# lhaippp/DMHomo

Measured on AMD Instinct MI355X. Metric: sampled images/sec (128x128, s_step=32), higher is better.
Workload: dtype f32; 1 GPU; DGM CFG-Unet dim=64 128x128 bs=25/GPU s_step=32 cond_scale=3 (BASELINE configs[1]); global_batch=25, cfg_mode=streams, hip_graph=True, weights=seeded random init

## Files before the change

### dmhomo_amd/csrc/attention.hip

```cpp
#include "common.h"

typedef float floatx16 __attribute__((ext_vector_type(16)));

#define LA_NS 128
#define LA_PART (32 + 32 + 1024)

__global__ __launch_bounds__(256) void linattn_context_kernel(const float* __restrict__ qkv,
                                                              float* __restrict__ partial, int n, int nsplit,
                                                              const int32_t* __restrict__ rows) {
  const int jb = blockIdx.x / nsplit, sp = blockIdx.x % nsplit;
  if (rows && jb >= rows[0]) return;
  const int b = dmh_rows_phys(rows, jb);
  const int lane = threadIdx.x & 63, h = threadIdx.x >> 6;
  const int d = lane & 31, half = lane >> 5;
  const int p0 = sp * LA_NS;
  const float* base = qkv + (size_t)b * n * 384;

  float kr[LA_NS / 2], vr[LA_NS / 2];
  const float* kp = base + (size_t)p0 * 384 + 128 + h * 32 + d + (size_t)half * 384;
#pragma unroll
  for (int i = 0; i < LA_NS / 2; ++i) {
    const int pix = p0 + 2 * i + half;
    const bool ok = pix < n;
    const float* q = ok ? kp + (size_t)i * 768 : kp;
    const float kv = q[0], vv = q[128];
    kr[i] = ok ? kv : -INFINITY;
    vr[i] = ok ? vv : 0.f;
  }
  float m = -INFINITY;
#pragma unroll
  for (int i = 0; i < LA_NS / 2; ++i) m = fmaxf(m, kr[i]);
  m = fmaxf(m, __shfl_xor(m, 32));
  float s = 0.f;
#pragma unroll
  for (int i = 0; i < LA_NS / 2; ++i) {
    kr[i] = __expf(kr[i] - m);
    s += kr[i];
  }
  s += __shfl_xor(s, 32);

  floatx16 acc;
#pragma unroll
  for (int r = 0; r < 16; ++r) acc[r] = 0.f;
#pragma unroll
  for (int i = 0; i < LA_NS / 2; ++i) acc = __builtin_amdgcn_mfma_f32_32x32x2f32(kr[i], vr[i], acc, 0, 0, 0);
  float* out = partial + ((size_t)(b * nsplit + sp) * 4 + h) * LA_PART;
  if (half == 0) {
    out[d] = m;
    out[32 + d] = s;
  }
#pragma unroll
  for (int r = 0; r < 16; ++r) {
    const int row = (r & 3) + 8 * (r >> 2) + 4 * half;
    out[64 + row * 32 + d] = acc[r];
  }
}

__global__ __launch_bounds__(1024) void linattn_merge_kernel(const float* __restrict__ partial,
                                                             float* __restrict__ ctx, int n, int nsplit,
                                                             float* __restrict__ ms, const int32_t* __restrict__ rows) {
  if (rows && (int)(blockIdx.x >> 2) >= rows[0]) return;
  const int b = dmh_rows_phys(rows, blockIdx.x >> 2), h = blockIdx.x & 3;
  const int bh = b * 4 + h;
  const int d = threadIdx.x >> 5, e = threadIdx.x & 31;
  const float* base = partial + ((size_t)b * nsplit * 4 + h) * LA_PART;
  const size_t stride = (size_t)4 * LA_PART;
  float M = -INFINITY;
#pragma unroll 8
  for (int sp = 0; sp < nsplit; ++sp) M = fmaxf(M, base[sp * stride + d]);
  float S = 0.f, acc = 0.f;
#pragma unroll 8
  for (int sp = 0; sp < nsplit; ++sp) {
    const float w = expf(base[sp * stride + d] - M);
    S = fmaf(base[sp * stride + 32 + d], w, S);
    acc = fmaf(base[sp * stride + 64 + d * 32 + e], w, acc);
  }
  ctx[(size_t)bh * 1024 + d * 32 + e] = acc / S / (float)n;
  if (ms && e == 0) {
    ms[((size_t)bh * 32 + d) * 2 + 0] = M;
    ms[((size_t)bh * 32 + d) * 2 + 1] = S;
  }
}

#define LA_TILES 4
__global__ __launch_bounds__(256) void linattn_apply_kernel(const float* __restrict__ qkv,
                                                            const float* __restrict__ ctx, float* __restrict__ out,
                                                            int n, int nblk, float scale,
                                                            const int32_t* __restrict__ rows) {
  const int jb = blockIdx.x / nblk, blk = blockIdx.x % nblk;
  if (rows && jb >= rows[0]) return;
  const int b = dmh_rows_phys(rows, jb);
  const int lane = threadIdx.x & 63, h = threadIdx.x >> 6;
  const int i = lane & 31, half = lane >> 5;
  const float* cb = ctx + ((size_t)(b * 4 + h)) * 1024;
  float bf[16];
#pragma unroll
  for (int s = 0; s < 16; ++s) bf[s] = cb[(half * 16 + s) * 32 + i];
  const float* base = qkv + (size_t)b * n * 384;
  float* ob = out + (size_t)b * n * 128;
  for (int tI = 0; tI < LA_TILES; ++tI) {
    const int p0 = (blk * LA_TILES + tI) * 32;
    if (p0 >= n) break;
    const int pix = p0 + i;
    float q[16];
    if (pix < n) {
      const float* qp = base + (size_t)pix * 384 + h * 32 + half * 16;
#pragma unroll
      for (int s4 = 0; s4 < 4; ++s4) {
        const float4 t = ld4(qp + s4 * 4);
        q[s4 * 4 + 0] = t.x;
        q[s4 * 4 + 1] = t.y;
        q[s4 * 4 + 2] = t.z;
        q[s4 * 4 + 3] = t.w;
      }
    } else {
#pragma unroll
      for (int s = 0; s < 16; ++s) q[s] = 0.f;
    }
    float m = q[0];
#pragma unroll
    for (int s = 1; s < 16; ++s) m = fmaxf(m, q[s]);
    m = fmaxf(m, __shfl_xor(m, 32));
    float sum = 0.f;
#pragma unroll
    for (int s = 0; s < 16; ++s) {
      q[s] = expf(q[s] - m);
      sum += q[s];
    }
    sum += __shfl_xor(sum, 32);
    floatx16 acc;
#pragma unroll
    for (int r = 0; r < 16; ++r) acc[r] = 0.f;
#pragma unroll
    for (int s = 0; s < 16; ++s) {
      const float a = (q[s] / sum) * scale;
      acc = __builtin_amdgcn_mfma_f32_32x32x2f32(a, bf[s], acc, 0, 0, 0);
    }
#pragma unroll
    for (int r = 0; r < 16; ++r) {
      const int row = (r & 3) + 8 * (r >> 2) + 4 * half;
      if (p0 + row < n) ob[(size_t)(p0 + row) * 128 + h * 32 + i] = acc[r];
    }
  }
}

__global__ __launch_bounds__(256) void attention_kernel(const float* __restrict__ qkv, float* __restrict__ out, int n,
                                                        int qtiles, float scale, const int32_t* __restrict__ rows) {
  const int wid = blockIdx.x * 4 + (threadIdx.x >> 6);
  const int lane = threadIdx.x & 63;
  const int i = lane & 31, half = lane >> 5;
  const int qt = wid % qtiles;
  const int bh = wid / qtiles;
  const int h = bh & 3;
  if (rows && (bh >> 2) >= rows[0]) return;
  const int b = dmh_rows_phys(rows, bh >> 2);
  const float* base = qkv + (size_t)b * n * 384;
  const int q0 = qt * 32;

  float qf[16];
  {
    const int qi = q0 + i;
    if (qi < n) {
      const float* qp = base + (size_t)qi * 384 + h * 32 + half * 16;
#pragma unroll
      for (int s4 = 0; s4 < 4; ++s4) {
        const float4 t = ld4(qp + s4 * 4);
        qf[s4 * 4 + 0] = t.x * scale;
        qf[s4 * 4 + 1] = t.y * scale;
        qf[s4 * 4 + 2] = t.z * scale;
        qf[s4 * 4 + 3] = t.w * scale;
      }
    } else {
#pragma unroll
      for (int s = 0; s < 16; ++s) qf[s] = 0.f;
    }
  }
  floatx16 oacc;
#pragma unroll
  for (int r = 0; r < 16; ++r) oacc[r] = 0.f;
  float mrun = -INFINITY, lrun = 0.f;

  for (int k0 = 0; k0 < n; k0 += 32) {
    float kf[16];
    const int ki = k0 + i;
    if (ki < n) {
      const float* kp = base + (size_t)ki * 384 + 128 + h * 32 + half * 16;
#pragma unroll
      for (int s4 = 0; s4 < 4; ++s4) {
        const float4 t = ld4(kp + s4 * 4);
        kf[s4 * 4 + 0] = t.x;
        kf[s4 * 4 + 1] = t.y;
        kf[s4 * 4 + 2] = t.z;
        kf[s4 * 4 + 3] = t.w;
      }
    } else {
#pragma unroll
      for (int s = 0; s < 16; ++s) kf[s] = 0.f;
    }
    floatx16 sacc;
#pragma unroll
    for (int r = 0; r < 16; ++r) sacc[r] = 0.f;
#pragma unroll
    for (int s = 0; s < 16; ++s) sacc = __builtin_amdgcn_mfma_f32_32x32x2f32(kf[s], qf[s], sacc, 0, 0, 0);
    float tmax = -INFINITY;
#pragma unroll
    for (int r = 0; r < 16; ++r) {
      const int key = k0 + (r & 3) + 8 * (r >> 2) + 4 * half;
      if (key >= n) sacc[r] = -INFINITY;
      tmax = fmaxf(tmax, sacc[r]);
    }
    tmax = fmaxf(tmax, __shfl_xor(tmax, 32));
    const float mnew = fmaxf(mrun, tmax);
    const float alpha = expf(mrun - mnew);
    float psum = 0.f;
#pragma unroll
    for (int r = 0; r < 16; ++r) {
      sacc[r] = expf(sacc[r] - mnew);
      psum += sacc[r];
    }
    psum += __shfl_xor(psum, 32);
    lrun = fmaf(lrun, alpha, psum);
    mrun = mnew;
#pragma unroll
    for (int r = 0; r < 16; ++r) oacc[r] *= alpha;
#pragma unroll
    for (int r = 0; r < 16; ++r) {
      const int key = k0 + (r & 3) + 8 * (r >> 2) + 4 * half;
      const float vv = (key < n) ? base[(size_t)key * 384 + 256 + h * 32 + i] : 0.f;
      oacc = __builtin_amdgcn_mfma_f32_32x32x2f32(vv, sacc[r], oacc, 0, 0, 0);
    }
  }
  const int qi = q0 + i;
  if (qi < n) {
    float* op = out + ((size_t)b * n + qi) * 128 + h * 32;
    const float inv = 1.0f / lrun;
#pragma unroll
    for (int g4 = 0; g4 < 4; ++g4) {
      float4 o;
      o.x = oacc[g4 * 4 + 0] * inv;
      o.y = oacc[g4 * 4 + 1] * inv;
      o.z = oacc[g4 * 4 + 2] * inv;
      o.w = oacc[g4 * 4 + 3] * inv;
      st4(op + 8 * g4 + 4 * half, o);
    }
  }
}

extern "C" int dmh_linattn_splits(int n) { return dmh_dims_ok({n}, 1, 1 << 26) ? cdiv(n, LA_NS) : -1; }

extern "C" int64_t dmh_linattn_partial_floats(int B, int n) {
  if (!dmh_dims_ok({B}) || !dmh_dims_ok({n}, 1, 1 << 26)) return -1;
  return (int64_t)B * dmh_linattn_splits(n) * 4 * LA_PART;
}

extern "C" int dmh_linattn_context(const float* qkv, float* partial, int B, int n, const int32_t* rows, void* stream) {
  DMH_REQUIRE(qkv && partial && B > 0 && n > 0, "dmh_linattn_context: bad arguments");
  const int ns = dmh_linattn_splits(n);
  hipLaunchKernelGGL(linattn_context_kernel, dim3(B * ns), dim3(256), 0, (hipStream_t)stream, qkv, partial, n, ns, rows);
  DMH_CHECK_LAUNCH("dmh_linattn_context");
  return DMH_OK;
}

extern "C" int dmh_linattn_merge(const float* partial, float* ctx, int B, int n, const int32_t* rows, void* stream) {
  DMH_REQUIRE(partial && ctx && B > 0 && n > 0, "dmh_linattn_merge: bad arguments");
  hipLaunchKernelGGL(linattn_merge_kernel, dim3(B * 4), dim3(1024), 0, (hipStream_t)stream, partial, ctx, n,
                     dmh_linattn_splits(n), (float*)nullptr, rows);
  DMH_CHECK_LAUNCH("dmh_linattn_merge");
  return DMH_OK;
}

extern "C" int dmh_linattn_merge_n(const float* partial, float* ctx, int B, int n, int nsplit, const int32_t* rows,
                                   void* stream) {
  DMH_REQUIRE(partial && ctx && B > 0 && n > 0 && nsplit > 0, "dmh_linattn_merge_n: bad arguments");
  hipLaunchKernelGGL(linattn_merge_kernel, dim3(B * 4), dim3(1024), 0, (hipStream_t)stream, partial, ctx, n, nsplit,
                     (float*)nullptr, rows);
  DMH_CHECK_LAUNCH("dmh_linattn_merge_n");
  return DMH_OK;
}

extern "C" int dmh_linattn_merge_ms(const float* partial, float* ctx, float* ms, int B, int n, void* stream) {
  DMH_REQUIRE(partial && ctx && ms && B > 0 && n > 0, "dmh_linattn_merge_ms: bad arguments");
  hipLaunchKernelGGL(linattn_merge_kernel, dim3(B * 4), dim3(1024), 0, (hipStream_t)stream, partial, ctx, n,
                     dmh_linattn_splits(n), ms, (const int32_t*)nullptr);
  DMH_CHECK_LAUNCH("dmh_linattn_merge_ms");
  return DMH_OK;
}

extern "C" int dmh_linattn_apply(const float* qkv, const float* ctx, float* out, int B, int n, float scale,
                                 const int32_t* rows, void* stream) {
  DMH_REQUIRE(qkv && ctx && out && B > 0 && n > 0, "dmh_linattn_apply: bad arguments");
  const int nblk = cdiv(n, 32 * LA_TILES);
  hipLaunchKernelGGL(linattn_apply_kernel, dim3(B * nblk), dim3(256), 0, (hipStream_t)stream, qkv, ctx, out, n, nblk,
                     scale, rows);
  DMH_CHECK_LAUNCH("dmh_linattn_apply");
  return DMH_OK;
}

extern "C" int dmh_attention(const float* qkv, float* out, int B, int n, float scale, const int32_t* rows, void* stream) {
  DMH_REQUIRE(qkv && out && B > 0 && n > 0, "dmh_attention: bad arguments");
  const int qtiles = cdiv(n, 32);
  const int waves = B * 4 * qtiles;
  hipLaunchKernelGGL(attention_kernel, dim3(waves / 4), dim3(256), 0, (hipStream_t)stream, qkv, out, n, qtiles, scale, rows);
  DMH_CHECK_LAUNCH("dmh_attention");
  return DMH_OK;
}
```

Baseline: 89.75 images/s.

## Stage K/V tiles in LDS shared by four query waves in attention

The attention kernel now groups four 32-query waves of the same batch-head into one workgroup. K and V for 256 keys are loaded cooperatively with vectorized float4 global loads into padded LDS, and every wave reuses them, so each wave no longer re-reads K and strided scalar V from global memory. The LDS stores are split into stages with barriers so compute on early stages can begin while later stages are still being written. The exchange is extra LDS use, since the launch raises the dynamic shared memory limit, plus block-wide barriers and a higher register count from holding the prefetched K/V.

```diff
diff --git a/dmhomo_amd/csrc/attention.hip b/dmhomo_amd/csrc/attention.hip
--- a/dmhomo_amd/csrc/attention.hip
+++ b/dmhomo_amd/csrc/attention.hip
@@ -1,3 +1,4 @@
+#include <algorithm>
 #include "common.h"
 
 typedef float floatx16 __attribute__((ext_vector_type(16)));
@@ -144,90 +145,137 @@
   }
 }
 
+#define AT_KB 256
+#define AT_KP 36
+#define AT_ROW (AT_KP + 32)
+#define AT_STAGES 4
+#define AT_SK (AT_KB / AT_STAGES)
+
+__device__ __forceinline__ float at_half_max(float v) {
+  unsigned o;
+  const unsigned a = dmh_xor32(__float_as_uint(v), &o);
+  return fmaxf(__uint_as_float(a), __uint_as_float(o));
+}
+__device__ __forceinline__ float at_half_sum(float v) {
+  unsigned o;
+  const unsigned a = dmh_xor32(__float_as_uint(v), &o);
+  return __uint_as_float(a) + __uint_as_float(o);
+}
+
+__device__ __forceinline__ void at_tile(const float* Ks, const float* Vs, int kt, int k0, int n, int i, int half,
+                                        const float (&qf)[16], floatx16& oacc, float& mrun, float& lrun) {
+  float kf[16];
+  const float* kp = Ks + (kt + i) * AT_KP + half * 16;
+#pragma unroll
+  for (int s4 = 0; s4 < 4; ++s4) {
+    const float4 t = ld4(kp + s4 * 4);
+    kf[s4 * 4 + 0] = t.x;
+    kf[s4 * 4 + 1] = t.y;
+    kf[s4 * 4 + 2] = t.z;
+    kf[s4 * 4 + 3] = t.w;
+  }
+  float vf[16];
+#pragma unroll
+  for (int r = 0; r < 16; ++r) vf[r] = Vs[(kt + (r & 3) + 8 * (r >> 2) + 4 * half) * 32 + i];
+  floatx16 sacc;
+#pragma unroll
+  for (int r = 0; r < 16; ++r) sacc[r] = 0.f;
+#pragma unroll
+  for (int s = 0; s < 16; ++s) sacc = __builtin_amdgcn_mfma_f32_32x32x2f32(kf[s], qf[s], sacc, 0, 0, 0);
+  float tmax = -INFINITY;
+#pragma unroll
+  for (int r = 0; r < 16; ++r) {
+    const int key = k0 + (r & 3) + 8 * (r >> 2) + 4 * half;
+    if (key >= n) sacc[r] = -INFINITY;
+    tmax = fmaxf(tmax, sacc[r]);
+  }
+  tmax = at_half_max(tmax);
+  const float mnew = fmaxf(mrun, tmax);
+  const float alpha = expf(mrun - mnew);
+  float psum = 0.f;
+#pragma unroll
+  for (int r = 0; r < 16; ++r) {
+    sacc[r] = expf(sacc[r] - mnew);
+    psum += sacc[r];
+  }
+  psum = at_half_sum(psum);
+  lrun = fmaf(lrun, alpha, psum);
+  mrun = mnew;
+#pragma unroll
+  for (int r = 0; r < 16; ++r) oacc[r] *= alpha;
+#pragma unroll
+  for (int r = 0; r < 16; ++r) oacc = __builtin_amdgcn_mfma_f32_32x32x2f32(vf[r], sacc[r], oacc, 0, 0, 0);
+}
+
 __global__ __launch_bounds__(256) void attention_kernel(const float* __restrict__ qkv, float* __restrict__ out, int n,
-                                                        int qtiles, float scale, const int32_t* __restrict__ rows) {
-  const int wid = blockIdx.x * 4 + (threadIdx.x >> 6);
-  const int lane = threadIdx.x & 63;
-  const int i = lane & 31, half = lane >> 5;
-  const int qt = wid % qtiles;
-  const int bh = wid / qtiles;
+                                                        int qblocks, float scale, const int32_t* __restrict__ rows) {
+  extern __shared__ __attribute__((aligned(16))) float at_smem[];
+  const int bh = blockIdx.x / qblocks, qb = blockIdx.x % qblocks;
   const int h = bh & 3;
   if (rows && (bh >> 2) >= rows[0]) return;
   const int b = dmh_rows_phys(rows, bh >> 2);
+  const int tid = threadIdx.x, lane = tid & 63;
+  const int i = lane & 31, half = lane >> 5;
   const float* base = qkv + (size_t)b * n * 384;
-  const int q0 = qt * 32;
+  const int q0 = (qb * 4 + (tid >> 6)) * 32;
+  const bool wave_on = q0 < n;
+  const int kcap = min(AT_KB, (n + 31) & ~31);
+  float* Ks = at_smem;
+  float* Vs = at_smem + kcap * AT_KP;
 
   float qf[16];
-  {
-    const int qi = q0 + i;
-    if (qi < n) {
-      const float* qp = base + (size_t)qi * 384 + h * 32 + half * 16;
-#pragma unroll
-      for (int s4 = 0; s4 < 4; ++s4) {
-        const float4 t = ld4(qp + s4 * 4);
-        qf[s4 * 4 + 0] = t.x * scale;
-        qf[s4 * 4 + 1] = t.y * scale;
-        qf[s4 * 4 + 2] = t.z * scale;
-        qf[s4 * 4 + 3] = t.w * scale;
-      }
-    } else {
-#pragma unroll
-      for (int s = 0; s < 16; ++s) qf[s] = 0.f;
-    }
-  }
+#pragma unroll
+  for (int s = 0; s < 16; ++s) qf[s] = 0.f;
   floatx16 oacc;
 #pragma unroll
   for (int r = 0; r < 16; ++r) oacc[r] = 0.f;
   float mrun = -INFINITY, lrun = 0.f;
 
-  for (int k0 = 0; k0 < n; k0 += 32) {
-    float kf[16];
-    const int ki = k0 + i;
-    if (ki < n) {
-      const float* kp = base + (size_t)ki * 384 + 128 + h * 32 + half * 16;
-#pragma unroll
-      for (int s4 = 0; s4 < 4; ++s4) {
-        const float4 t = ld4(kp + s4 * 4);
-        kf[s4 * 4 + 0] = t.x;
-        kf[s4 * 4 + 1] = t.y;
-        kf[s4 * 4 + 2] = t.z;
-        kf[s4 * 4 + 3] = t.w;
+  for (int kb0 = 0; kb0 < n; kb0 += AT_KB) {
+    const int kleft = n - kb0;
+    const int kcnt = min(AT_KB, (kleft + 31) & ~31);
+    float4 kreg[AT_KB / 32], vreg[AT_KB / 32];
+#pragma unroll
+    for (int j = 0; j < AT_KB / 32; ++j) {
+      const int key = j * 32 + (tid >> 3);
+      const bool ok = key < kleft;
+      const float* gp = base + (size_t)(kb0 + (ok ? key : 0)) * 384 + 128 + h * 32 + (tid & 7) * 4;
+      const float4 kv = ld4(gp), vv = ld4(gp + 128);
+      kreg[j] = make_float4(ok ? kv.x : 0.f, ok ? kv.y : 0.f, ok ? kv.z : 0.f, ok ? kv.w : 0.f);
+      vreg[j] = make_float4(ok ? vv.x : 0.f, ok ? vv.y : 0.f, ok ? vv.z : 0.f, ok ? vv.w : 0.f);
+      if (j == AT_SK / 32 - 1 && kb0 == 0 && q0 + i < n) {
+        const float* qp = base + (size_t)(q0 + i) * 384 + h * 32 + half * 16;
+#pragma unroll
+        for (int s4 = 0; s4 < 4; ++s4) {
+          const float4 t = ld4(qp + s4 * 4);
+          qf[s4 * 4 + 0] = t.x;
+          qf[s4 * 4 + 1] = t.y;
+          qf[s4 * 4 + 2] = t.z;
+          qf[s4 * 4 + 3] = t.w;
+        }
       }
-    } else {
-#pragma unroll
-      for (int s = 0; s < 16; ++s) kf[s] = 0.f;
-    }
-    floatx16 sacc;
-#pragma unroll
-    for (int r = 0; r < 16; ++r) sacc[r] = 0.f;
-#pragma unroll
-    for (int s = 0; s < 16; ++s) sacc = __builtin_amdgcn_mfma_f32_32x32x2f32(kf[s], qf[s], sacc, 0, 0, 0);
-    float tmax = -INFINITY;
-#pragma unroll
-    for (int r = 0; r < 16; ++r) {
-      const int key = k0 + (r & 3) + 8 * (r >> 2) + 4 * half;
-      if (key >= n) sacc[r] = -INFINITY;
-      tmax = fmaxf(tmax, sacc[r]);
-    }
-    tmax = fmaxf(tmax, __shfl_xor(tmax, 32));
-    const float mnew = fmaxf(mrun, tmax);
-    const float alpha = expf(mrun - mnew);
-    float psum = 0.f;
-#pragma unroll
-    for (int r = 0; r < 16; ++r) {
-      sacc[r] = expf(sacc[r] - mnew);
-      psum += sacc[r];
-    }
-    psum += __shfl_xor(psum, 32);
-    lrun = fmaf(lrun, alpha, psum);
-    mrun = mnew;
-#pragma unroll
-    for (int r = 0; r < 16; ++r) oacc[r] *= alpha;
-#pragma unroll
-    for (int r = 0; r < 16; ++r) {
-      const int key = k0 + (r & 3) + 8 * (r >> 2) + 4 * half;
-      const float vv = (key < n) ? base[(size_t)key * 384 + 256 + h * 32 + i] : 0.f;
-      oacc = __builtin_amdgcn_mfma_f32_32x32x2f32(vv, sacc[r], oacc, 0, 0, 0);
+    }
+    if (kb0) __syncthreads();
+#pragma unroll
+    for (int st = 0; st < AT_STAGES; ++st) {
+      if (st * AT_SK >= kcnt) break;
+#pragma unroll
+      for (int j = st * (AT_SK / 32); j < (st + 1) * (AT_SK / 32); ++j) {
+        const int key = j * 32 + (tid >> 3);
+        if (key < kcnt) {
+          st4(Ks + key * AT_KP + (tid & 7) * 4, kreg[j]);
+          st4(Vs + key * 32 + (tid & 7) * 4, vreg[j]);
+        }
+      }
+      __syncthreads();
+      if (wave_on) {
+        if (st == 0 && kb0 == 0) {
+#pragma unroll
+          for (int s = 0; s < 16; ++s) qf[s] *= scale;
+        }
+        const int kend = min(kcnt, (st + 1) * AT_SK);
+        for (int kt = st * AT_SK; kt < kend; kt += 32) at_tile(Ks, Vs, kt, kb0 + kt, n, i, half, qf, oacc, mrun, lrun);
+      }
     }
   }
   const int qi = q0 + i;
@@ -298,9 +346,13 @@
 
 extern "C" int dmh_attention(const float* qkv, float* out, int B, int n, float scale, const int32_t* rows, void* stream) {
   DMH_REQUIRE(qkv && out && B > 0 && n > 0, "dmh_attention: bad arguments");
-  const int qtiles = cdiv(n, 32);
-  const int waves = B * 4 * qtiles;
-  hipLaunchKernelGGL(attention_kernel, dim3(waves / 4), dim3(256), 0, (hipStream_t)stream, qkv, out, n, qtiles, scale, rows);
+  DMH_REQUIRE(dmh_dims_ok({B}) && dmh_dims_ok({n}), "dmh_attention: B and n must lie in (0, 2^20]");
+  const int qblocks = cdiv(n, 128);
+  DMH_REQUIRE((int64_t)B * 4 * qblocks <= 0x7fffffff, "dmh_attention: too many workgroups");
+  const int lds = std::min(AT_KB, (n + 31) & ~31) * AT_ROW * (int)sizeof(float);
+  DMH_RAISE_LDS_ONCE(attention_kernel, AT_KB * AT_ROW * sizeof(float), "dmh_attention");
+  hipLaunchKernelGGL(attention_kernel, dim3(B * 4 * qblocks), dim3(256), lds, (hipStream_t)stream, qkv, out, n, qblocks,
+                     scale, rows);
   DMH_CHECK_LAUNCH("dmh_attention");
   return DMH_OK;
 }
```

New measurement: 90.57 images/s, median of 6. About the same (+0.9%).
